# nabeelre/BTSbot

Hardware: AMD Instinct MI355X
Metric: alerts/sec (63×63×3 triplet + 25 meta) train+infer, 1/2/4/8 MI355X (higher is better)
Workload: dtype bf16; 1 GPU; BASELINE.json configs[1]: ConvNeXt-pico multi-modal (mm_ConvNeXt) bf16 inference, batch=1024 synthetic triplets per GPU, inputs resident in HBM, logits+scores out; per_gpu_batch=1024, global_batch=1024, precision=bf16, weights=seeded random, layer-scale ~1, parallelism=1 independent replicas, batch-sharded, no collective, pipeline_depth=3

## Files before the change

### btsbot_amd/csrc/stage1b.hip

```cpp
#include "common.h"
#include "stage0.h"
#include <type_traits>

namespace {

typedef __attribute__((ext_vector_type(16))) float f32x16;
typedef __attribute__((address_space(1))) const void* gptr_t;
typedef __attribute__((address_space(3))) void* lptr_t;

template <typename T> struct SCM;
typedef __attribute__((ext_vector_type(4))) short s16x4;
typedef __attribute__((ext_vector_type(4))) _Float16 f16x4;
template <> struct SCM<bf16_t> {
  using frag = bf16x8;
  using frag4 = s16x4;
  static __device__ __forceinline__ f32x16 run(frag a, frag b, f32x16 c) {
    return __builtin_amdgcn_mfma_f32_32x32x16_bf16(a, b, c, 0, 0, 0);
  }
  static __device__ __forceinline__ f32x4 run4(frag4 a, frag4 b, f32x4 c) {
    return __builtin_amdgcn_mfma_f32_4x4x4bf16_1k(a, b, c, 0, 0, 0);
  }
};
template <> struct SCM<f16_t> {
  using frag = f16x8;
  using frag4 = f16x4;
  static __device__ __forceinline__ f32x16 run(frag a, frag b, f32x16 c) {
    return __builtin_amdgcn_mfma_f32_32x32x16_f16(a, b, c, 0, 0, 0);
  }
  static __device__ __forceinline__ f32x4 run4(frag4 a, frag4 b, f32x4 c) {
    return __builtin_amdgcn_mfma_f32_4x4x4f16(a, b, c, 0, 0, 0);
  }
};

constexpr int C = 128, HW = 7, PA = 49, G = 2, NPX = G * PA, CT = 4, HID = 512, KS1 = 8;
constexpr int CN = 256, PO = 9;
constexpr int PITCH = 2 * C + 16;
constexpr int MAPB = NPX * PITCH;
constexpr int CHUNKB = 16384, HALFB = CHUNKB / 2, NCH = HID / 32, NSLOT = 3;
constexpr int PL_ROW = 136 * 8, PL_XQ = 8 * PL_ROW, PL_AL = 2 * PL_XQ, PLB = G * PL_AL;
constexpr int OFF_PL = 2 * CHUNKB;
template <bool X2> struct S1L {
  static constexpr int PLANES = X2 ? 2 : 1;
  static constexpr int SLB = X2 ? 2 * HALFB : HALFB;
  static constexpr int OFF_W2X = OFF_PL + PLANES * PLB;
  static constexpr int OFF_B1 = OFF_W2X + (X2 ? 2 * SLB : 0);
  static constexpr int OFF_PART = OFF_B1 + (HID + C) * 4;
  static constexpr int OFF_ST = OFF_PART + 2 * 4 * 128 * 4;
  static constexpr int LDS_BYTES = OFF_ST + 2 * 128 * 4;
  static_assert(4 * SLB <= PLANES * PLB, "W1 slots + W2 slot 0 inside the planar images");
};
static_assert(MAPB <= 2 * CHUNKB && S1L<false>::LDS_BYTES <= 80 * 1024 && S1L<true>::LDS_BYTES <= 160 * 1024, "LDS layout");
constexpr float LN_EPS = 1e-6f;
constexpr int TW_R = 21, TW_BYTES = TW_R * C * 4 * 4 * 2;
constexpr int PARB = TW_BYTES + 3 * C * 4;
constexpr int PARB_X2 = 2 * TW_BYTES + 3 * C * 4;

#define SC_STAMP(i)                                                                \
  do {                                                                             \
    if (a.stamps != nullptr && blockIdx.x == 0 && threadIdx.x == 0) a.stamps[i] = clock64(); \
    if (a.wgt != nullptr && threadIdx.x == 0 && ((i) == 0 || (i) == 13))           \
      a.wgt[2 * blockIdx.x + ((i) == 13)] = wall_clock64();                        \
  } while (0)

template <int N> __device__ __forceinline__ void wait_vm() {
  asm volatile("s_waitcnt vmcnt(%0)" ::"n"(N) : "memory");
}
__device__ __forceinline__ int swz4(int row) {
  return (4 - ((row >> 2) & 3)) & 3;
}
__device__ __forceinline__ float swap_add32(float a, float b) {
  auto r = __builtin_amdgcn_permlane32_swap(__float_as_uint(a), __float_as_uint(b), false, false);
  return __uint_as_float(r[0]) + __uint_as_float(r[1]);
}
__device__ __forceinline__ float swap_add16(float a, float b) {
  auto r = __builtin_amdgcn_permlane16_swap(__float_as_uint(a), __float_as_uint(b), false, false);
  return __uint_as_float(r[0]) + __uint_as_float(r[1]);
}
template <int CTRL> __device__ __forceinline__ float dpp_mov(float v) {
  return __builtin_bit_cast(float, __builtin_amdgcn_update_dpp(0, __builtin_bit_cast(int, v), CTRL, 0xF, 0xF, true));
}
__device__ __forceinline__ void block_reduce32(float (&w)[32], int lane, float (&out)[2]) {
#pragma unroll
  for (int n = 0; n < 16; ++n) w[n] = swap_add32(w[n], w[n + 16]);
#pragma unroll
  for (int n = 0; n < 8; ++n) w[n] = swap_add16(w[n], w[n + 8]);
  const bool b3 = (lane & 8) != 0, b2 = (lane & 4) != 0;
#pragma unroll
  for (int n = 0; n < 4; ++n) {
    const float own = b3 ? w[n + 4] : w[n], send = b3 ? w[n] : w[n + 4];
    w[n] = own + dpp_mov<0x128>(send);
  }
#pragma unroll
  for (int n = 0; n < 2; ++n) {
    const float own = b2 ? w[n + 2] : w[n], send = b2 ? w[n] : w[n + 2];
    const float lo = dpp_mov<0x124>(send), hi = dpp_mov<0x12C>(send);
    out[n] = own + (b2 ? lo : hi);
  }
}

__device__ __forceinline__ void ln_regs(const f32x16 (&x)[CT], const float* __restrict__ w,
                                        const float* __restrict__ b, int h, f32x16 (&y)[CT]) {
  float s = 0.f;
#pragma unroll
  for (int ct = 0; ct < CT; ++ct)
#pragma unroll
    for (int r = 0; r < 16; ++r) s += x[ct][r];
  s += __shfl_xor(s, 32, 64);
  const float mean = s * (1.0f / C);
  float q = 0.f;
#pragma unroll
  for (int ct = 0; ct < CT; ++ct)
#pragma unroll
    for (int r = 0; r < 16; ++r) {
      const float d = x[ct][r] - mean;
      q += d * d;
    }
  q += __shfl_xor(q, 32, 64);
  const float rstd = rsqrtf(q * (1.0f / C) + LN_EPS);
#pragma unroll
  for (int ct = 0; ct < CT; ++ct)
#pragma unroll
    for (int qd = 0; qd < 4; ++qd) {
      const int c = ct * 32 + 8 * qd + 4 * h;
      const float4 wv = *reinterpret_cast<const float4*>(w + c);
      const float4 bv = *reinterpret_cast<const float4*>(b + c);
      y[ct][4 * qd + 0] = (x[ct][4 * qd + 0] - mean) * rstd * wv.x + bv.x;
      y[ct][4 * qd + 1] = (x[ct][4 * qd + 1] - mean) * rstd * wv.y + bv.y;
      y[ct][4 * qd + 2] = (x[ct][4 * qd + 2] - mean) * rstd * wv.z + bv.z;
      y[ct][4 * qd + 3] = (x[ct][4 * qd + 3] - mean) * rstd * wv.w + bv.w;
    }
}

template <typename T, int LOPLANE = 0>
__device__ __forceinline__ void regs_to_map(const f32x16 (&x)[CT], unsigned char* map, int p, int h) {
  typedef T __attribute__((ext_vector_type(4))) T4;
#pragma unroll
  for (int ct = 0; ct < CT; ++ct)
#pragma unroll
    for (int qd = 0; qd < 4; ++qd) {
      T4 v, w;
#pragma unroll
      for (int e = 0; e < 4; ++e) {
        v[e] = (T)x[ct][4 * qd + e];
        if (LOPLANE > 0) w[e] = (T)(x[ct][4 * qd + e] - (float)v[e]);
      }
      *reinterpret_cast<T4*>(map + p * PITCH + (ct * 32 + 8 * qd + 4 * h) * 2) = v;
      if (LOPLANE > 0) *reinterpret_cast<T4*>(map + LOPLANE + p * PITCH + (ct * 32 + 8 * qd + 4 * h) * 2) = w;
    }
}

template <typename T, int LOPLANE = 0, bool SAT = false>
__device__ __forceinline__ void regs_to_planar(const f32x16 (&x)[CT], unsigned char* pl, int p, int h) {
  const int al = p >= PA ? 1 : 0, pp = p - al * PA;
  const int y = pp / HW, xx = pp - y * HW;
  unsigned char* dst = pl + al * PL_AL + (xx >> 2) * PL_XQ + y * PL_ROW + (xx & 3) * 2 + h * 32;
#pragma unroll
  for (int ct = 0; ct < CT; ++ct)
#pragma unroll
    for (int r = 0; r < 16; ++r) {
      const T hi = (T)(SAT ? __builtin_amdgcn_fmed3f(x[ct][r], -65504.0f, 65504.0f) : x[ct][r]);
      *reinterpret_cast<T*>(dst + (ct * 32 + 8 * (r >> 2) + (r & 3)) * 8) = hi;
      if (LOPLANE > 0) *reinterpret_cast<T*>(dst + LOPLANE + (ct * 32 + 8 * (r >> 2) + (r & 3)) * 8) = (T)(x[ct][r] - (float)hi);
    }
}

template <typename T, bool X2, int WPS = 2, bool KEEP = false>
__global__ __launch_bounds__(256, WPS) void stage1b_kernel(Stage1Args a) {
  using frag = typename SCM<T>::frag;
  using DT = typename std::conditional<KEEP, f16_t, T>::type;
  using frag4 = typename SCM<DT>::frag4;
  extern __shared__ __attribute__((aligned(16))) unsigned char smem[];
  unsigned char* pl = smem + OFF_PL;
  unsigned char* stg = smem;
  using L = S1L<X2>;
  constexpr int SLB = L::SLB;
  constexpr int PLO = X2 ? PLB : 0;
  float* b1s = reinterpret_cast<float*>(smem + L::OFF_B1);
  float* b2s = b1s + HID;
  float* part = reinterpret_cast<float*>(smem + L::OFF_PART);
  float* st = reinterpret_cast<float*>(smem + L::OFF_ST);
  auto w1slot = [&](int sl) { return pl + sl * SLB; };
  auto w2slot = [&](int sl) { return sl == 0 ? pl + 3 * SLB : (X2 ? smem + L::OFF_W2X : smem) + (sl - 1) * SLB; };

  const int tid = threadIdx.x, lane = tid & 63, wave = __builtin_amdgcn_readfirstlane(tid >> 6);
  const int lr = lane & 31, h = lane >> 5;
  const bool w1wave = wave < 2;
  const int a0 = blockIdx.x * G;
  const int nal = min(G, a.B - a0);
  const int p = wave * 32 + lr;
  const bool live = p < nal * PA;
  const bool inmap = p < NPX;
  const int pm = inmap ? p : 0;
  SC_STAMP(0);
  auto zero_pads = [&]() {
#pragma unroll
    for (int pn = 0; pn < L::PLANES; ++pn) {
      unsigned char* pb = pl + pn * PLB;
      for (int i = tid; i < 4 * PL_ROW / 16; i += 256) {
        const int blk = i / (PL_ROW / 16), o = i - blk * (PL_ROW / 16);
        *reinterpret_cast<uint4*>(pb + (blk >> 1) * PL_AL + (blk & 1) * PL_XQ + 7 * PL_ROW + o * 16) = make_uint4(0u, 0u, 0u, 0u);
      }
      for (int i = tid; i < G * HW * C; i += 256) {
        const int al = i / (HW * C), r = (i / C) % HW, c = i % C;
        *reinterpret_cast<unsigned short*>(pb + al * PL_AL + PL_XQ + r * PL_ROW + c * 8 + 6) = 0;
      }
    }
  };
  zero_pads();
  const float* xsrc = a.x_in + ((size_t)a0 * PA + (live ? p : 0)) * C;
  float* xscr = a.scratch + ((size_t)a0 * PA + (live ? p : 0)) * C;
  auto load_x = [&](const float* src, f32x16 (&x)[CT]) {
#pragma unroll
    for (int ct = 0; ct < CT; ++ct)
#pragma unroll
      for (int qd = 0; qd < 4; ++qd) {
        const float4 v4 = *reinterpret_cast<const float4*>(src + ct * 32 + 8 * qd + 4 * h);
        x[ct][4 * qd + 0] = live ? v4.x : 0.f;
        x[ct][4 * qd + 1] = live ? v4.y : 0.f;
        x[ct][4 * qd + 2] = live ? v4.z : 0.f;
        x[ct][4 * qd + 3] = live ? v4.w : 0.f;
      }
  };
  {
    f32x16 x0[CT];
    load_x(xsrc, x0);
    if (inmap) regs_to_planar<DT, PLO, KEEP && !std::is_same<T, f16_t>::value>(x0, pl, p, h);
  }
  SC_STAMP(1);

  f32x16 x[CT];
  const int rot = (blockIdx.x * 5 + (blockIdx.x >> 4)) & (NCH - 1);
#pragma unroll
  for (int j = 0; j < 2; ++j) {
    const Stage0Blk& bk = a.blk[j];
    int ln = lane;
    asm volatile("" : "+v"(ln));
    const int dj = ln & 3, db = ln >> 2;
    const float b1v0 = bk.b1[tid], b1v1 = bk.b1[256 + tid];
    const float b2v = bk.gamma[tid & (C - 1)] * bk.b2[tid & (C - 1)];
    const uint2* twsrc = reinterpret_cast<const uint2*>(bk.par) + (2 * wave) * 64 + ln;
    frag4 tw[TW_R], twl[X2 ? TW_R : 1];
#pragma unroll
    for (int r = 0; r < TW_R; ++r) tw[r] = __builtin_bit_cast(frag4, twsrc[r * 512]);
    if (X2) {
#pragma unroll
      for (int r = 0; r < TW_R; ++r) twl[r] = __builtin_bit_cast(frag4, twsrc[TW_BYTES / 8 + r * 512]);
    }
    const float* pf = reinterpret_cast<const float*>(bk.par + (X2 ? 2 : 1) * TW_BYTES);
    float dwbias[2], lng[2], lnb2[2];
#pragma unroll
    for (int gi = 0; gi < 2; ++gi) {
      const int c = 16 * (2 * wave + gi) + db;
      dwbias[gi] = pf[c];
      lng[gi] = pf[C + c];
      lnb2[gi] = pf[2 * C + c];
    }
    SC_STAMP(2 + 5 * j);
    __syncthreads();
    b1s[tid] = b1v0;
    b1s[256 + tid] = b1v1;
    if (tid < C) b2s[tid] = b2v;

    const unsigned char* wsrc[4];
    const unsigned char* wsrcl[4];
#pragma unroll
    for (int i = 0; i < 4; ++i) {
      const int pc = wave * 4 + i;
      if (pc < 8) {
        const int m = pc * 4 + (lane >> 4);
        const int hid = (m & ~12) | ((m & 4) << 1) | ((m & 8) >> 1);
        const size_t o = (size_t)hid * (C * 2) + (((lane & 15) ^ (m & 15)) << 4);
        wsrc[i] = bk.w1 + o;
        wsrcl[i] = X2 ? bk.w1_lo + o : nullptr;
      } else {
        const int r = (pc - 8) * 16 + (lane >> 2);
        const size_t o = (size_t)r * (HID * 2) + (((lane & 3) ^ swz4(r)) << 4);
        wsrc[i] = bk.w2g + o;
        wsrcl[i] = X2 ? bk.w2g_lo + o : nullptr;
      }
    }
    const int wstep0 = w1wave ? 32 * C * 2 : 64;
    auto issue = [&](int k) {
      unsigned char* dst = (w1wave ? w1slot(k % NSLOT) : w2slot(k % NSLOT)) + (wave & 1) * 4096;
#pragma unroll
      for (int i = 0; i < 4; ++i)
        __builtin_amdgcn_global_load_lds((gptr_t)(wsrc[i] + (size_t)((k + rot) & (NCH - 1)) * wstep0),
                                         (lptr_t)(dst + i * 1024), 16, 0, 0);
      if (X2) {
#pragma unroll
        for (int i = 0; i < 4; ++i)
          __builtin_amdgcn_global_load_lds((gptr_t)(wsrcl[i] + (size_t)((k + rot) & (NCH - 1)) * wstep0),
                                           (lptr_t)(dst + HALFB + i * 1024), 16, 0, 0);
      }
    };
    auto issue_piece = [&](int k, int i) {
      unsigned char* dst = (w1wave ? w1slot(k % NSLOT) : w2slot(k % NSLOT)) + (wave & 1) * 4096;
      if (X2 && i >= 4)
        __builtin_amdgcn_global_load_lds((gptr_t)(wsrcl[i & 3] + (size_t)((k + rot) & (NCH - 1)) * wstep0),
                                         (lptr_t)(dst + HALFB + (i & 3) * 1024), 16, 0, 0);
      else
        __builtin_amdgcn_global_load_lds((gptr_t)(wsrc[i] + (size_t)((k + rot) & (NCH - 1)) * wstep0),
                                         (lptr_t)(dst + i * 1024), 16, 0, 0);
    };
    SC_STAMP(3 + 5 * j);

    int rofs[11];
#pragma unroll
    for (int sx = 0; sx < 11; ++sx) {
      const int r = sx + dj - 3;
      rofs[sx] = ((unsigned)r < (unsigned)HW ? r : 7) * PL_ROW;
    }
    float v[2][2][16];
#pragma unroll
    for (int gi = 0; gi < 2; ++gi) {
      if (gi == 1) {
#pragma unroll
        for (int r = 0; r < TW_R; ++r) tw[r] = __builtin_bit_cast(frag4, twsrc[r * 512 + 64]);
        if (X2) {
#pragma unroll
          for (int r = 0; r < TW_R; ++r) twl[r] = __builtin_bit_cast(frag4, twsrc[TW_BYTES / 8 + r * 512 + 64]);
        }
      }
      f32x4 acc[G][2][2];
#pragma unroll
      for (int al = 0; al < G; ++al)
#pragma unroll
        for (int yb = 0; yb < 2; ++yb)
#pragma unroll
          for (int xb = 0; xb < 2; ++xb) acc[al][yb][xb] = f32x4{dwbias[gi], dwbias[gi], dwbias[gi], dwbias[gi]};
      const unsigned char* lb = pl + (16 * (2 * wave + gi) + db) * 8;
      frag4 bq[2][G][2], bql[X2 ? 2 : 1][G][X2 ? 2 : 1];
      auto read_step = [&](int sx, int buf) {
#pragma unroll
        for (int al = 0; al < G; ++al)
#pragma unroll
          for (int q = 0; q < 2; ++q) {
            bq[buf][al][q] = __builtin_bit_cast(frag4, *reinterpret_cast<const uint2*>(lb + al * PL_AL + q * PL_XQ + rofs[sx]));
            if (X2)
              bql[buf][al][q] =
                  __builtin_bit_cast(frag4, *reinterpret_cast<const uint2*>(lb + PLB + al * PL_AL + q * PL_XQ + rofs[sx]));
          }
      };
      read_step(0, 0);
#ifdef S1_EXP_NODW
#pragma unroll 1
      for (int sx = 0; sx < 0; ++sx) {
#else
#pragma unroll
      for (int sx = 0; sx < 11; ++sx) {
#endif
#pragma unroll
        for (int al = 0; al < G; ++al)
#pragma unroll
          for (int q = 0; q < 2; ++q) {
            asm volatile("" : "+v"(bq[sx & 1][al][q]));
            if (X2) asm volatile("" : "+v"(bql[X2 ? sx & 1 : 0][al][X2 ? q : 0]));
          }
        if (sx + 1 < 11) read_step(sx + 1, (sx + 1) & 1);
        __builtin_amdgcn_sched_barrier(0);
#pragma unroll
        for (int al = 0; al < G; ++al)
#pragma unroll
          for (int yb = 0; yb < 2; ++yb) {
            const int ky = sx - 4 * yb;
            if (ky < 0 || ky > 6) continue;
#pragma unroll
            for (int rbi = 0; rbi < 3; ++rbi)
#pragma unroll
              for (int xb = 0; xb < 2; ++xb) {
                const int q = xb + rbi - 1;
                if (q < 0 || q > 1) continue;
                if (X2) {
                  acc[al][yb][xb] = SCM<DT>::run4(twl[ky * 3 + rbi], bq[sx & 1][al][q], acc[al][yb][xb]);
                  acc[al][yb][xb] = SCM<DT>::run4(tw[ky * 3 + rbi], bql[X2 ? sx & 1 : 0][al][X2 ? q : 0], acc[al][yb][xb]);
                }
                acc[al][yb][xb] = SCM<DT>::run4(tw[ky * 3 + rbi], bq[sx & 1][al][q], acc[al][yb][xb]);
              }
          }
        __builtin_amdgcn_sched_barrier(0);
      }
#pragma unroll
      for (int al = 0; al < G; ++al)
#pragma unroll
        for (int yb = 0; yb < 2; ++yb)
#pragma unroll
          for (int xb = 0; xb < 2; ++xb)
#pragma unroll
            for (int i = 0; i < 4; ++i) v[gi][al][yb * 8 + xb * 4 + i] = acc[al][yb][xb][i];
    }
    if (KEEP && a.keep_d[j] != nullptr) {
#pragma unroll
      for (int gi = 0; gi < 2; ++gi)
#pragma unroll
        for (int al = 0; al < G; ++al) {
          if (al >= nal) continue;
          float* dst = a.keep_d[j] + (size_t)(a0 + al) * PA * C + 16 * (2 * wave + gi) + db;
#pragma unroll
          for (int yb = 0; yb < 2; ++yb)
#pragma unroll
            for (int xb = 0; xb < 2; ++xb)
              if (yb < 1 || dj < 3) {
#pragma unroll
                for (int i = 0; i < 4; ++i) {
                  if (xb == 1 && i == 3) continue;
                  dst[((4 * yb + dj) * HW + 4 * xb + i) * C] = v[gi][al][yb * 8 + xb * 4 + i];
                }
              }
        }
    }
    SC_STAMP(4 + 5 * j);
    {
      float o1[2], o2[2];
      {
        float s1[32];
#pragma unroll
        for (int al = 0; al < G; ++al)
#pragma unroll
          for (int n = 0; n < 16; ++n) s1[al * 16 + n] = v[0][al][n] + v[1][al][n];
        block_reduce32(s1, ln, o1);
      }
      {
        float s2[32];
#pragma unroll
        for (int al = 0; al < G; ++al)
#pragma unroll
          for (int n = 0; n < 16; ++n) s2[al * 16 + n] = fmaf(v[0][al][n], v[0][al][n], v[1][al][n] * v[1][al][n]);
        block_reduce32(s2, ln, o2);
      }
      const int slot = (ln >> 5) * 64 + (4 * ((ln >> 4) & 1) + dj) * 8 + 4 * ((ln >> 3) & 1) + 2 * ((ln >> 2) & 1);
      *reinterpret_cast<float2*>(part + wave * 128 + slot) = make_float2(o1[0], o1[1]);
      *reinterpret_cast<float2*>(part + 512 + wave * 128 + slot) = make_float2(o2[0], o2[1]);
    }
    __syncthreads();
    if (tid < 128) {
      const float t1 = part[tid] + part[128 + tid] + part[256 + tid] + part[384 + tid];
      const float t2 = part[512 + tid] + part[640 + tid] + part[768 + tid] + part[896 + tid];
      const float mean = t1 * (1.0f / C);
      const float rstd = rsqrtf(fmaxf(t2 * (1.0f / C) - mean * mean, 0.0f) + LN_EPS);
      st[tid] = rstd;
      st[128 + tid] = -mean * rstd;
    }
    __syncthreads();
    auto write_ln = [&](bool lo_pass) {
#pragma unroll
      for (int gi = 0; gi < 2; ++gi) {
        T* mo = reinterpret_cast<T*>(stg) + 16 * (2 * wave + gi) + db;
#pragma unroll
        for (int al = 0; al < G; ++al)
#pragma unroll
          for (int yb = 0; yb < 2; ++yb)
#pragma unroll
            for (int xb = 0; xb < 2; ++xb) {
              const int slot = al * 64 + (4 * yb + dj) * 8 + 4 * xb;
              const float4 r4 = *reinterpret_cast<const float4*>(st + slot);
              const float4 m4 = *reinterpret_cast<const float4*>(st + 128 + slot);
              const float rr[4] = {r4.x, r4.y, r4.z, r4.w}, mm[4] = {m4.x, m4.y, m4.z, m4.w};
              if (yb < 1 || dj < 3) {
#pragma unroll
                for (int i = 0; i < 4; ++i) {
                  if (xb == 1 && i == 3) continue;
                  const float y = fmaf(fmaf(v[gi][al][yb * 8 + xb * 4 + i], rr[i], mm[i]), lng[gi], lnb2[gi]);
                  const T yh = (T)y;
                  mo[(al * PA + (4 * yb + dj) * HW + 4 * xb + i) * (PITCH / 2)] = lo_pass ? (T)(y - (float)yh) : yh;
                }
              }
            }
      }
    };
    write_ln(false);
    __syncthreads();
    if (KEEP) {
      unsigned char* dst = reinterpret_cast<unsigned char*>(a.keep_xn[j]) + (size_t)a0 * PA * C * 2;
      for (int i = tid; i < nal * PA * 16; i += 256) {
        const int pp = i >> 4, c16 = i & 15;
        *reinterpret_cast<uint4*>(dst + (size_t)pp * C * 2 + 16 * c16) = *reinterpret_cast<const uint4*>(stg + pp * PITCH + 16 * c16);
      }
    }
    issue(0);
    SC_STAMP(5 + 5 * j);

    load_x(j == 0 ? xsrc : xscr, x);
    {
      frag xf[KS1], xfl[X2 ? KS1 : 1];
#pragma unroll
      for (int ks = 0; ks < KS1; ++ks)
        xf[ks] = *reinterpret_cast<const frag*>(stg + pm * PITCH + ks * 32 + h * 16);
      if (X2) {
        __syncthreads();
        write_ln(true);
        __syncthreads();
#pragma unroll
        for (int ks = 0; ks < KS1; ++ks)
          xfl[ks] = *reinterpret_cast<const frag*>(stg + pm * PITCH + ks * 32 + h * 16);
      }
#pragma unroll
      for (int ct = 0; ct < CT; ++ct)
#pragma unroll
        for (int qd = 0; qd < 4; ++qd) {
          const float4 bv = *reinterpret_cast<const float4*>(b2s + ct * 32 + 8 * qd + 4 * h);
          x[ct][4 * qd + 0] += bv.x;
          x[ct][4 * qd + 1] += bv.y;
          x[ct][4 * qd + 2] += bv.z;
          x[ct][4 * qd + 3] += bv.w;
        }
      asm volatile("s_waitcnt lgkmcnt(0)" ::: "memory");
      __syncthreads();
      issue(1);
      if (w1wave) issue(2);
      auto bias_acc = [&](int k, f32x16& acc) {
        const float* bp = b1s + ((k + rot) & (NCH - 1)) * 32 + 8 * h;
#pragma unroll
        for (int qd = 0; qd < 4; ++qd) {
          const f32x4 bv = __builtin_bit_cast(f32x4, *reinterpret_cast<const bf16x8*>(bp + 4 * (qd & 1) + 16 * (qd >> 1)));
#pragma unroll
          for (int e = 0; e < 4; ++e) acc[4 * qd + e] = bv[e];
        }
      };
      frag a1l[X2 ? KS1 : 1];
      auto read_a1 = [&](int k, frag (&a1)[KS1]) {
        const unsigned char* w1s = w1slot(k % NSLOT);
#pragma unroll
        for (int ks = 0; ks < KS1; ++ks) {
          a1[ks] = *reinterpret_cast<const frag*>(w1s + lr * 256 + (((ks * 2 + h) ^ (lr & 15)) << 4));
          if (X2) a1l[ks] = *reinterpret_cast<const frag*>(w1s + HALFB + lr * 256 + (((ks * 2 + h) ^ (lr & 15)) << 4));
        }
      };
#ifdef S1_LOOPSTAMP
      unsigned long long lts[16];
#define LS(i) do { __builtin_amdgcn_sched_barrier(0); if (ch == 6 || ch == 7) lts[i + 8 * (ch - 6)] = __builtin_amdgcn_s_memtime(); __builtin_amdgcn_sched_barrier(0); } while (0)
#else
#define LS(i)
#endif
      f32x16 hacc[2];
      frag a1[KS1];
      {
        wait_vm<X2 ? 8 : 4>();
        asm volatile("s_waitcnt lgkmcnt(0)" ::: "memory");
        __builtin_amdgcn_s_barrier();
        bias_acc(0, hacc[0]);
        read_a1(0, a1);
#pragma unroll
        for (int ks = 0; ks < KS1; ++ks) {
          if (X2) {
            hacc[0] = SCM<T>::run(a1l[ks], xf[ks], hacc[0]);
            hacc[0] = SCM<T>::run(a1[ks], xfl[ks], hacc[0]);
          }
          hacc[0] = SCM<T>::run(a1[ks], xf[ks], hacc[0]);
        }
        __builtin_amdgcn_sched_barrier(0);
        wait_vm<0>();
        asm volatile("s_waitcnt lgkmcnt(0)" ::: "memory");
        __builtin_amdgcn_s_barrier();
        bias_acc(1, hacc[1]);
        read_a1(1, a1);
        if (w1wave) issue(3);
      }
      auto step = [&](auto last_c, int ch, f32x16& hc, f32x16& hn) {
        constexpr bool LAST = decltype(last_c)::value;
        LS(0);
        wait_vm<X2 ? 8 : 4>();
        LS(1);
        asm volatile("s_waitcnt lgkmcnt(0)" ::: "memory");
#ifndef S1_EXP_NOBAR
        __builtin_amdgcn_s_barrier();
#endif
        LS(2);
        frag a2[CT][2], a2l[X2 ? CT : 1][2];
        const unsigned char* w2s = w2slot(ch % NSLOT);
#pragma unroll
        for (int ct = 0; ct < CT; ++ct)
#pragma unroll
          for (int s2 = 0; s2 < 2; ++s2) {
            const int r = ct * 32 + lr;
            a2[ct][s2] = *reinterpret_cast<const frag*>(w2s + r * 64 + (((s2 * 2 + h) ^ swz4(r)) << 4));
            if (X2) a2l[ct][s2] = *reinterpret_cast<const frag*>(w2s + HALFB + r * 64 + (((s2 * 2 + h) ^ swz4(r)) << 4));
          }
        LS(3);
        const int kdma = ch + (w1wave ? 4 : 2);
        __builtin_amdgcn_sched_barrier(0);
        LS(4);
        float g[16];
#pragma unroll
        for (int r = 0; r < 8; ++r) {
          if (!LAST) {
            if (X2) {
              hn = SCM<T>::run(a1l[r], xf[r], hn);
              hn = SCM<T>::run(a1[r], xfl[r], hn);
            }
            hn = SCM<T>::run(a1[r], xf[r], hn);
          }
#ifdef S1_EXP_NOGELU
          g[r] = hc[r];
#else
          g[r] = gelu_for<T>(hc[r]);
#endif
#ifndef S1_EXP_NODMA
          if (X2) issue_piece(kdma, r);
          else if (r & 1) issue_piece(kdma, r >> 1);
#endif
          __builtin_amdgcn_sched_barrier(0);
        }
        LS(5);
        if (!LAST) read_a1(ch + 2, a1);
        frag hf, hfl;
#pragma unroll
        for (int r = 0; r < 8; ++r) {
          hf[r] = (T)g[r];
          if (X2) hfl[r] = (T)(g[r] - (float)hf[r]);
        }
#pragma unroll
        for (int ct = 0; ct < CT; ++ct) {
          if (X2) {
            x[ct] = SCM<T>::run(a2l[ct][0], hf, x[ct]);
            x[ct] = SCM<T>::run(a2[ct][0], hfl, x[ct]);
          }
          x[ct] = SCM<T>::run(a2[ct][0], hf, x[ct]);
#ifdef S1_EXP_NOGELU
          g[8 + 2 * ct] = hc[8 + 2 * ct];
          g[9 + 2 * ct] = hc[9 + 2 * ct];
#else
          g[8 + 2 * ct] = gelu_for<T>(hc[8 + 2 * ct]);
          g[9 + 2 * ct] = gelu_for<T>(hc[9 + 2 * ct]);
#endif
          __builtin_amdgcn_sched_barrier(0);
        }
        if (!LAST) bias_acc(ch + 2, hc);
#pragma unroll
        for (int r = 0; r < 8; ++r) {
          hf[r] = (T)g[8 + r];
          if (X2) hfl[r] = (T)(g[8 + r] - (float)hf[r]);
        }
        LS(6);
#pragma unroll
        for (int ct = 0; ct < CT; ++ct) {
          if (X2) {
            x[ct] = SCM<T>::run(a2l[ct][1], hf, x[ct]);
            x[ct] = SCM<T>::run(a2[ct][1], hfl, x[ct]);
          }
          x[ct] = SCM<T>::run(a2[ct][1], hf, x[ct]);
        }
        LS(7);
      };
#ifndef S1_EXP_NOLOOP
#pragma unroll 1
      for (int ch = 0; ch < NCH - 2; ch += 2) {
        step(std::false_type{}, ch, hacc[0], hacc[1]);
        step(std::false_type{}, ch + 1, hacc[1], hacc[0]);
      }
      step(std::false_type{}, NCH - 2, hacc[0], hacc[1]);
      step(std::true_type{}, NCH - 1, hacc[1], hacc[0]);
#endif
      asm volatile("s_waitcnt lgkmcnt(0)" ::: "memory");
#ifdef S1_LOOPSTAMP
      if (a.wgt != nullptr && blockIdx.x == 0 && tid == 0 && j == 0)
        for (int i = 0; i < 16; ++i) a.wgt[4096 + i] = lts[i];
#endif
      wait_vm<0>();
      if (j == 0) {
        __syncthreads();
        zero_pads();
        if (inmap) regs_to_planar<DT, PLO, KEEP && !std::is_same<T, f16_t>::value>(x, pl, p, h);
        if (live) {
#pragma unroll
          for (int ct = 0; ct < CT; ++ct)
#pragma unroll
            for (int qd = 0; qd < 4; ++qd)
              *reinterpret_cast<float4*>(xscr + ct * 32 + 8 * qd + 4 * h) =
                  make_float4(x[ct][4 * qd], x[ct][4 * qd + 1], x[ct][4 * qd + 2], x[ct][4 * qd + 3]);
        }
      }
    }
    SC_STAMP(6 + 5 * j);
  }
  if (a.tap_stage != nullptr && live) {
    float* tp = a.tap_stage + ((size_t)a0 * PA + p) * C;
#pragma unroll
    for (int ct = 0; ct < CT; ++ct)
#pragma unroll
      for (int qd = 0; qd < 4; ++qd)
        *reinterpret_cast<float4*>(tp + ct * 32 + 8 * qd + 4 * h) =
            make_float4(x[ct][4 * qd], x[ct][4 * qd + 1], x[ct][4 * qd + 2], x[ct][4 * qd + 3]);
  }

  {
    __syncthreads();
    {
      f32x16 xn[CT];
      ln_regs(x, a.ds_lnw, a.ds_lnb, h, xn);
      if (inmap) regs_to_map<T, X2 ? MAPB : 0>(xn, stg, p, h);
    }
    static_assert(2 * MAPB <= L::OFF_B1, "two [pixel][channel] images in front of the bias words");
    constexpr int KSD = 4 * C / 16, RING = X2 ? 8 : 16, NSTEP = 2 * KSD;
    const frag* wsrc = reinterpret_cast<const frag*>(a.ds_w) + lane;
    auto fsrc = [&](int stp) {
      return wsrc + (size_t)((wave + 4 * (stp >> 5)) * KSD + (stp & (KSD - 1))) * (X2 ? 128 : 64);
    };
    frag wq[RING], wql[X2 ? RING : 1];
#pragma unroll
    for (int i = 0; i < RING; ++i) {
      wq[i] = *fsrc(i);
      if (X2) wql[i] = fsrc(i)[64];
    }
    __syncthreads();
    if (KEEP) {
      unsigned char* dst = reinterpret_cast<unsigned char*>(a.keep_patches) + (size_t)a0 * PO * 4 * C * 2;
      for (int i = tid; i < nal * PO * 4 * 16; i += 256) {
        const int c16 = i & 15, q = (i >> 4) & 3, o2 = i >> 6;
        const int g2 = o2 / PO, oo2 = o2 - g2 * PO;
        const int pin2 = g2 * PA + (2 * (oo2 / 3) + (q >> 1)) * HW + 2 * (oo2 % 3) + (q & 1);
        *reinterpret_cast<uint4*>(dst + (size_t)(o2 * 4 + q) * C * 2 + 16 * c16) =
            *reinterpret_cast<const uint4*>(stg + pin2 * PITCH + 16 * c16);
      }
    }
    SC_STAMP(12);
    const int o = lr;
    const bool olive = o < nal * PO;
    const int oc = o < G * PO ? o : 0;
    const int g = oc / PO, oo = oc - g * PO;
    const int oy = oo / 3, ox = oo - oy * 3;
    f32x16 acc;
    constexpr int RPT = KSD / RING;
#ifdef S1_EXP_NODS
#pragma unroll 1
    for (int rd = 0; rd < 0; ++rd) {
#else
#pragma unroll 1
    for (int rd = 0; rd < NSTEP / RING; ++rd) {
#endif
      const int cot = wave + 4 * (rd / RPT);
      if (rd % RPT == 0) {
#pragma unroll
        for (int qd = 0; qd < 4; ++qd) {
          const float4 bv = *reinterpret_cast<const float4*>(a.ds_b + cot * 32 + 8 * qd + 4 * h);
          acc[4 * qd + 0] = bv.x;
          acc[4 * qd + 1] = bv.y;
          acc[4 * qd + 2] = bv.z;
          acc[4 * qd + 3] = bv.w;
        }
      }
#pragma unroll
      for (int i = 0; i < RING; ++i) {
        const int stp = rd * RING + i, ks = stp & (KSD - 1);
        const int q = ks >> 3;
        const int pin = g * PA + (2 * oy + (q >> 1)) * HW + 2 * ox + (q & 1);
        const frag bf = *reinterpret_cast<const frag*>(stg + pin * PITCH + (ks & 7) * 32 + h * 16);
        if (X2) {
          const frag bfl = *reinterpret_cast<const frag*>(stg + MAPB + pin * PITCH + (ks & 7) * 32 + h * 16);
          acc = SCM<T>::run(wql[i], bf, acc);
          acc = SCM<T>::run(wq[i], bfl, acc);
        }
        acc = SCM<T>::run(wq[i], bf, acc);
        if (stp + RING < NSTEP) {
          wq[i] = *fsrc(stp + RING);
          if (X2) wql[i] = fsrc(stp + RING)[64];
        }
      }
      if (rd % RPT == RPT - 1 && olive) {
        float* dst = a.out + ((size_t)a0 * PO + o) * CN + cot * 32 + 4 * h;
#pragma unroll
        for (int qd = 0; qd < 4; ++qd)
          *reinterpret_cast<float4*>(dst + 8 * qd) =
              make_float4(acc[4 * qd], acc[4 * qd + 1], acc[4 * qd + 2], acc[4 * qd + 3]);
      }
    }
    SC_STAMP(13);
  }
}

template <typename T, bool X2>
__global__ void pack_s1par_kernel(const float* __restrict__ taps, const float* __restrict__ dw_b,
                                  const float* __restrict__ ln_w, const float* __restrict__ ln_b,
                                  unsigned char* __restrict__ out) {
  const int idx = blockIdx.x * blockDim.x + threadIdx.x;
  constexpr int NTW = TW_R * C * 16;
  if (idx < NTW) {
    const int k = idx & 3, i = (idx >> 2) & 3, c = (idx >> 4) & (C - 1), r = idx / (16 * C);
    const int ky = r / 3, rb = r % 3 - 1, kx = 4 * rb + k - i + 3;
    const float w = (kx >= 0 && kx < 7) ? taps[(ky * 7 + kx) * C + c] : 0.f;
    const T wh = (T)w;
    reinterpret_cast<T*>(out)[idx] = wh;
    if (X2) reinterpret_cast<T*>(out)[NTW + idx] = (T)(w - (float)wh);
    return;
  }
  const int f = idx - NTW;
  if (f >= 3 * C) return;
  float v;
  if (f < C) v = dw_b[f];
  else if (f < 2 * C) v = ln_w[f - C];
  else v = ln_b[f - 2 * C];
  reinterpret_cast<float*>(out + (X2 ? 2 : 1) * TW_BYTES)[f] = v;
}

template <typename T, bool X2 = false>
__global__ void pack_frag32_kernel(const float* __restrict__ w, T* __restrict__ out, int rows, int cin) {
  const long i = (long)blockIdx.x * blockDim.x + threadIdx.x;
  const int K = 4 * cin;
  if (i >= (long)rows * K) return;
  const int j = (int)(i & 7), l = (int)((i >> 3) & 63);
  const long fs = i >> 9;
  const int ksteps = K / 16;
  const int sk = (int)(fs % ksteps), tile = (int)(fs / ksteps);
  const int row = 32 * tile + (l & 31), k = 16 * sk + 8 * (l >> 5) + j;
  const int q = k / cin, c = k - q * cin;
  const float v = w[((long)row * cin + c) * 4 + q];
  const T vh = (T)v;
  if (X2) {
    out[fs * 1024 + l * 8 + j] = vh;
    out[fs * 1024 + 512 + l * 8 + j] = (T)(v - (float)vh);
  } else {
    out[i] = vh;
  }
}

template <typename T, bool X2 = false, int WPS = 2, bool KEEP = false> int launch_stage1b_t(const Stage1Args& a, hipStream_t st) {
  auto kern = stage1b_kernel<T, X2, WPS, KEEP>;
  static DevOnce attr_set;
  static const int pad = switch_on(SW_S1_ONE_WG) && !X2 ? 90 * 1024 - S1L<X2>::LDS_BYTES : 0;
  const int LDS_BYTES = S1L<X2>::LDS_BYTES + pad;
  if (attr_set.need()) {
    HIP_TRY(hipFuncSetAttribute(reinterpret_cast<const void*>(kern),
                                hipFuncAttributeMaxDynamicSharedMemorySize, (int)LDS_BYTES));
    attr_set.done();
  }
  hipLaunchKernelGGL(kern, dim3((a.B + G - 1) / G), dim3(256), LDS_BYTES, st, a);
  LAUNCH_CHECK();
  return BTSBOT_OK;
}

}

#ifdef STAGE1B_X2_TU
int launch_stage1b_x2(const Stage1Args& a, hipStream_t st) {
  if (a.blk[0].w1_lo == nullptr || a.blk[0].w2g_lo == nullptr || a.blk[1].w1_lo == nullptr || a.blk[1].w2g_lo == nullptr) {
    btsbot_set_error("stage1b: the split mode needs the filters' remainder images (w1_lo, w2g_lo)");
    return BTSBOT_ERR_INVALID_ARG;
  }
  return launch_stage1b_t<f16_t, true, 1>(a, st);
}
int launch_pack_s1par_x2(const float* taps, const float* dw_b, const float* ln_w, const float* ln_b, void* out,
                         hipStream_t st) {
  const dim3 grid((TW_R * C * 16 + 3 * C + 255) / 256), blk(256);
  hipLaunchKernelGGL((pack_s1par_kernel<f16_t, true>), grid, blk, 0, st, taps, dw_b, ln_w, ln_b,
                     reinterpret_cast<unsigned char*>(out));
  LAUNCH_CHECK();
  return BTSBOT_OK;
}
int launch_pack_frag32_x2(const float* src, void* dst, int cout, int cin, hipStream_t st) {
  const long total = (long)cout * 4 * cin;
  hipLaunchKernelGGL((pack_frag32_kernel<f16_t, true>), dim3((unsigned)((total + 255) / 256)), dim3(256), 0, st, src,
                     reinterpret_cast<f16_t*>(dst), cout, cin);
  LAUNCH_CHECK();
  return BTSBOT_OK;
}
#else
int launch_stage1b_x2(const Stage1Args& a, hipStream_t st);
int launch_pack_s1par_x2(const float* taps, const float* dw_b, const float* ln_w, const float* ln_b, void* out,
                         hipStream_t st);
int launch_pack_frag32_x2(const float* src, void* dst, int cout, int cin, hipStream_t st);

size_t s1par_bytes() { return PARB_X2; }

int launch_pack_s1par(int prec, const float* taps, const float* dw_b, const float* ln_w,
                      const float* ln_b, void* out, hipStream_t st) {
  unsigned char* o = reinterpret_cast<unsigned char*>(out);
  const dim3 grid((TW_R * C * 16 + 3 * C + 255) / 256), blk(256);
  if (prec == BTSBOT_BF16)
    hipLaunchKernelGGL((pack_s1par_kernel<bf16_t, false>), grid, blk, 0, st, taps, dw_b, ln_w, ln_b, o);
  else if (prec == BTSBOT_F16)
    hipLaunchKernelGGL((pack_s1par_kernel<f16_t, false>), grid, blk, 0, st, taps, dw_b, ln_w, ln_b, o);
  else if (prec == BTSBOT_F16X2)
    return launch_pack_s1par_x2(taps, dw_b, ln_w, ln_b, out, st);
  else {
    btsbot_set_error("pack_s1par: precision %d is not a 16-bit mode", prec);
    return BTSBOT_ERR_INVALID_ARG;
  }
  LAUNCH_CHECK();
  return BTSBOT_OK;
}

int launch_pack_frag32(int prec, const float* src, void* dst, int cout, int cin, hipStream_t st) {
  const long total = (long)cout * 4 * cin;
  const dim3 grid((unsigned)((total + 255) / 256)), blk(256);
  if (prec == BTSBOT_BF16)
    hipLaunchKernelGGL(pack_frag32_kernel<bf16_t>, grid, blk, 0, st, src, reinterpret_cast<bf16_t*>(dst), cout, cin);
  else if (prec == BTSBOT_F16)
    hipLaunchKernelGGL(pack_frag32_kernel<f16_t>, grid, blk, 0, st, src, reinterpret_cast<f16_t*>(dst), cout, cin);
  else if (prec == BTSBOT_F16X2)
    return launch_pack_frag32_x2(src, dst, cout, cin, st);
  else {
    btsbot_set_error("pack_frag32: precision %d is not a 16-bit mode", prec);
    return BTSBOT_ERR_INVALID_ARG;
  }
  LAUNCH_CHECK();
  return BTSBOT_OK;
}

bool stage1_supported(int prec, int c1, int c2) {
  return (prec == BTSBOT_BF16 || prec == BTSBOT_F16 || prec == BTSBOT_F16X2) && c1 == 128 && c2 == 256;
}

int launch_stage1b(int prec, const Stage1Args& a, hipStream_t st) {
  if (a.B <= 0) return BTSBOT_OK;
  if (a.keep_xn[0] != nullptr) {
    if ((a.keep_d[0] == nullptr) != (a.keep_d[1] == nullptr) || a.keep_xn[1] == nullptr || a.keep_patches == nullptr ||
        a.tap_stage == nullptr || a.scratch == nullptr) {
      btsbot_set_error("stage1b: the training forward needs every kept buffer");
      return BTSBOT_ERR_INVALID_ARG;
    }
    if (prec == BTSBOT_BF16) return launch_stage1b_t<bf16_t, false, 2, true>(a, st);
    if (prec == BTSBOT_F16) return launch_stage1b_t<f16_t, false, 2, true>(a, st);
    btsbot_set_error("stage1b: the training forward runs in the bf16 / f16 modes, not %d", prec);
    return BTSBOT_ERR_INVALID_ARG;
  }
  if (prec == BTSBOT_BF16) return launch_stage1b_t<bf16_t>(a, st);
  if (prec == BTSBOT_F16) return launch_stage1b_t<f16_t>(a, st);
  if (prec == BTSBOT_F16X2) return launch_stage1b_x2(a, st);
  btsbot_set_error("stage1b: unsupported precision %d", prec);
  return BTSBOT_ERR_INVALID_ARG;
}
#endif
```

Baseline: 3.637 million alerts/s.

## Move ConvNeXt LayerNorm into per-pixel registers after fp32 LDS transpose

The depthwise-conv output is no longer reduced across lanes with permlane/DPP and a partial-sum table. It is now written as an fp32 image into LDS, reusing the ring slots and planar area. Each lane reads back its pixel's 64 channels and computes mean and variance in registers, then builds the bf16 MFMA fragments and the optional low-precision residual fragments directly. This removes extra barriers and the staging write/read of normalized activations. The residual x load is deferred and overlapped with the first W1 chunk by raising the vmcnt wait threshold, and LN weights move to LDS. In exchange it writes and reads a larger fp32 image in LDS, raises register pressure (64 floats plus 16 float4 per lane), and uses two-pass variance instead of E[x²]-mean².

```diff
diff --git a/btsbot_amd/csrc/stage1b.hip b/btsbot_amd/csrc/stage1b.hip
--- a/btsbot_amd/csrc/stage1b.hip
+++ b/btsbot_amd/csrc/stage1b.hip
@@ -39,17 +39,18 @@
 constexpr int CHUNKB = 16384, HALFB = CHUNKB / 2, NCH = HID / 32, NSLOT = 3;
 constexpr int PL_ROW = 136 * 8, PL_XQ = 8 * PL_ROW, PL_AL = 2 * PL_XQ, PLB = G * PL_AL;
 constexpr int OFF_PL = 2 * CHUNKB;
+constexpr int LNP = 4 * C + 16;
 template <bool X2> struct S1L {
   static constexpr int PLANES = X2 ? 2 : 1;
   static constexpr int SLB = X2 ? 2 * HALFB : HALFB;
   static constexpr int OFF_W2X = OFF_PL + PLANES * PLB;
   static constexpr int OFF_B1 = OFF_W2X + (X2 ? 2 * SLB : 0);
-  static constexpr int OFF_PART = OFF_B1 + (HID + C) * 4;
-  static constexpr int OFF_ST = OFF_PART + 2 * 4 * 128 * 4;
-  static constexpr int LDS_BYTES = OFF_ST + 2 * 128 * 4;
+  static constexpr int OFF_LNW = OFF_B1 + (HID + C) * 4;
+  static constexpr int LDS_BYTES = OFF_LNW + 2 * C * 4;
   static_assert(4 * SLB <= PLANES * PLB, "W1 slots + W2 slot 0 inside the planar images");
+  static_assert(NPX * LNP <= OFF_PL + PLB && NPX * LNP <= OFF_B1, "the fp32 image lies in ring slots 0, 1 + the planar image");
 };
-static_assert(MAPB <= 2 * CHUNKB && S1L<false>::LDS_BYTES <= 80 * 1024 && S1L<true>::LDS_BYTES <= 160 * 1024, "LDS layout");
+static_assert(MAPB <= 2 * CHUNKB && S1L<false>::LDS_BYTES <= 75264 && S1L<true>::LDS_BYTES <= 160 * 1024, "LDS layout");
 constexpr float LN_EPS = 1e-6f;
 constexpr int TW_R = 21, TW_BYTES = TW_R * C * 4 * 4 * 2;
 constexpr int PARB = TW_BYTES + 3 * C * 4;
@@ -68,36 +69,6 @@
 __device__ __forceinline__ int swz4(int row) {
   return (4 - ((row >> 2) & 3)) & 3;
 }
-__device__ __forceinline__ float swap_add32(float a, float b) {
-  auto r = __builtin_amdgcn_permlane32_swap(__float_as_uint(a), __float_as_uint(b), false, false);
-  return __uint_as_float(r[0]) + __uint_as_float(r[1]);
-}
-__device__ __forceinline__ float swap_add16(float a, float b) {
-  auto r = __builtin_amdgcn_permlane16_swap(__float_as_uint(a), __float_as_uint(b), false, false);
-  return __uint_as_float(r[0]) + __uint_as_float(r[1]);
-}
-template <int CTRL> __device__ __forceinline__ float dpp_mov(float v) {
-  return __builtin_bit_cast(float, __builtin_amdgcn_update_dpp(0, __builtin_bit_cast(int, v), CTRL, 0xF, 0xF, true));
-}
-__device__ __forceinline__ void block_reduce32(float (&w)[32], int lane, float (&out)[2]) {
-#pragma unroll
-  for (int n = 0; n < 16; ++n) w[n] = swap_add32(w[n], w[n + 16]);
-#pragma unroll
-  for (int n = 0; n < 8; ++n) w[n] = swap_add16(w[n], w[n + 8]);
-  const bool b3 = (lane & 8) != 0, b2 = (lane & 4) != 0;
-#pragma unroll
-  for (int n = 0; n < 4; ++n) {
-    const float own = b3 ? w[n + 4] : w[n], send = b3 ? w[n] : w[n + 4];
-    w[n] = own + dpp_mov<0x128>(send);
-  }
-#pragma unroll
-  for (int n = 0; n < 2; ++n) {
-    const float own = b2 ? w[n + 2] : w[n], send = b2 ? w[n] : w[n + 2];
-    const float lo = dpp_mov<0x124>(send), hi = dpp_mov<0x12C>(send);
-    out[n] = own + (b2 ? lo : hi);
-  }
-}
-
 __device__ __forceinline__ void ln_regs(const f32x16 (&x)[CT], const float* __restrict__ w,
                                         const float* __restrict__ b, int h, f32x16 (&y)[CT]) {
   float s = 0.f;
@@ -177,8 +148,8 @@
   constexpr int PLO = X2 ? PLB : 0;
   float* b1s = reinterpret_cast<float*>(smem + L::OFF_B1);
   float* b2s = b1s + HID;
-  float* part = reinterpret_cast<float*>(smem + L::OFF_PART);
-  float* st = reinterpret_cast<float*>(smem + L::OFF_ST);
+  float* lnws = reinterpret_cast<float*>(smem + L::OFF_LNW);
+  float* lnbs = lnws + C;
   auto w1slot = [&](int sl) { return pl + sl * SLB; };
   auto w2slot = [&](int sl) { return sl == 0 ? pl + 3 * SLB : (X2 ? smem + L::OFF_W2X : smem) + (sl - 1) * SLB; };
 
@@ -191,6 +162,7 @@
   const bool live = p < nal * PA;
   const bool inmap = p < NPX;
   const int pm = inmap ? p : 0;
+  const int lnrow = pm * LNP + h * 32;
   SC_STAMP(0);
   auto zero_pads = [&]() {
 #pragma unroll
@@ -247,19 +219,16 @@
       for (int r = 0; r < TW_R; ++r) twl[r] = __builtin_bit_cast(frag4, twsrc[TW_BYTES / 8 + r * 512]);
     }
     const float* pf = reinterpret_cast<const float*>(bk.par + (X2 ? 2 : 1) * TW_BYTES);
-    float dwbias[2], lng[2], lnb2[2];
-#pragma unroll
-    for (int gi = 0; gi < 2; ++gi) {
-      const int c = 16 * (2 * wave + gi) + db;
-      dwbias[gi] = pf[c];
-      lng[gi] = pf[C + c];
-      lnb2[gi] = pf[2 * C + c];
-    }
+    float dwbias[2];
+#pragma unroll
+    for (int gi = 0; gi < 2; ++gi) dwbias[gi] = pf[16 * (2 * wave + gi) + db];
+    const float lnv = pf[C + tid];
     SC_STAMP(2 + 5 * j);
     __syncthreads();
     b1s[tid] = b1v0;
     b1s[256 + tid] = b1v1;
     if (tid < C) b2s[tid] = b2v;
+    lnws[tid] = lnv;
 
     const unsigned char* wsrc[4];
     const unsigned char* wsrcl[4];
@@ -409,104 +378,86 @@
         }
     }
     SC_STAMP(4 + 5 * j);
+    __syncthreads();
     {
-      float o1[2], o2[2];
-      {
-        float s1[32];
+      unsigned char* dst = smem + dj * (HW * LNP) + (32 * wave + db) * 4;
+#pragma unroll
+      for (int gi = 0; gi < 2; ++gi)
 #pragma unroll
         for (int al = 0; al < G; ++al)
 #pragma unroll
-          for (int n = 0; n < 16; ++n) s1[al * 16 + n] = v[0][al][n] + v[1][al][n];
-        block_reduce32(s1, ln, o1);
-      }
-      {
-        float s2[32];
-#pragma unroll
-        for (int al = 0; al < G; ++al)
-#pragma unroll
-          for (int n = 0; n < 16; ++n) s2[al * 16 + n] = fmaf(v[0][al][n], v[0][al][n], v[1][al][n] * v[1][al][n]);
-        block_reduce32(s2, ln, o2);
-      }
-      const int slot = (ln >> 5) * 64 + (4 * ((ln >> 4) & 1) + dj) * 8 + 4 * ((ln >> 3) & 1) + 2 * ((ln >> 2) & 1);
-      *reinterpret_cast<float2*>(part + wave * 128 + slot) = make_float2(o1[0], o1[1]);
-      *reinterpret_cast<float2*>(part + 512 + wave * 128 + slot) = make_float2(o2[0], o2[1]);
-    }
-    __syncthreads();
-    if (tid < 128) {
-      const float t1 = part[tid] + part[128 + tid] + part[256 + tid] + part[384 + tid];
-      const float t2 = part[512 + tid] + part[640 + tid] + part[768 + tid] + part[896 + tid];
-      const float mean = t1 * (1.0f / C);
-      const float rstd = rsqrtf(fmaxf(t2 * (1.0f / C) - mean * mean, 0.0f) + LN_EPS);
-      st[tid] = rstd;
-      st[128 + tid] = -mean * rstd;
-    }
-    __syncthreads();
-    auto write_ln = [&](bool lo_pass) {
-#pragma unroll
-      for (int gi = 0; gi < 2; ++gi) {
-        T* mo = reinterpret_cast<T*>(stg) + 16 * (2 * wave + gi) + db;
-#pragma unroll
-        for (int al = 0; al < G; ++al)
-#pragma unroll
           for (int yb = 0; yb < 2; ++yb)
 #pragma unroll
-            for (int xb = 0; xb < 2; ++xb) {
-              const int slot = al * 64 + (4 * yb + dj) * 8 + 4 * xb;
-              const float4 r4 = *reinterpret_cast<const float4*>(st + slot);
-              const float4 m4 = *reinterpret_cast<const float4*>(st + 128 + slot);
-              const float rr[4] = {r4.x, r4.y, r4.z, r4.w}, mm[4] = {m4.x, m4.y, m4.z, m4.w};
+            for (int xb = 0; xb < 2; ++xb)
               if (yb < 1 || dj < 3) {
 #pragma unroll
                 for (int i = 0; i < 4; ++i) {
                   if (xb == 1 && i == 3) continue;
-                  const float y = fmaf(fmaf(v[gi][al][yb * 8 + xb * 4 + i], rr[i], mm[i]), lng[gi], lnb2[gi]);
-                  const T yh = (T)y;
-                  mo[(al * PA + (4 * yb + dj) * HW + 4 * xb + i) * (PITCH / 2)] = lo_pass ? (T)(y - (float)yh) : yh;
+                  const int col = 4 * xb + i, ofs = (al * PA + 4 * yb * HW + col) * LNP + gi * 64;
+                  *reinterpret_cast<float*>(dst + ofs) = v[gi][al][yb * 8 + xb * 4 + i];
                 }
               }
-            }
-      }
-    };
-    write_ln(false);
+    }
     __syncthreads();
-    if (KEEP) {
-      unsigned char* dst = reinterpret_cast<unsigned char*>(a.keep_xn[j]) + (size_t)a0 * PA * C * 2;
-      for (int i = tid; i < nal * PA * 16; i += 256) {
-        const int pp = i >> 4, c16 = i & 15;
-        *reinterpret_cast<uint4*>(dst + (size_t)pp * C * 2 + 16 * c16) = *reinterpret_cast<const uint4*>(stg + pp * PITCH + 16 * c16);
-      }
-    }
-    issue(0);
-    SC_STAMP(5 + 5 * j);
-
-    load_x(j == 0 ? xsrc : xscr, x);
+
     {
+      auto lds4 = [](const void* q) { return __builtin_bit_cast(f32x4, *reinterpret_cast<const bf16x8*>(q)); };
       frag xf[KS1], xfl[X2 ? KS1 : 1];
+      float xv[64];
 #pragma unroll
       for (int ks = 0; ks < KS1; ++ks)
-        xf[ks] = *reinterpret_cast<const frag*>(stg + pm * PITCH + ks * 32 + h * 16);
-      if (X2) {
-        __syncthreads();
-        write_ln(true);
-        __syncthreads();
-#pragma unroll
-        for (int ks = 0; ks < KS1; ++ks)
-          xfl[ks] = *reinterpret_cast<const frag*>(stg + pm * PITCH + ks * 32 + h * 16);
-      }
-#pragma unroll
-      for (int ct = 0; ct < CT; ++ct)
-#pragma unroll
-        for (int qd = 0; qd < 4; ++qd) {
-          const float4 bv = *reinterpret_cast<const float4*>(b2s + ct * 32 + 8 * qd + 4 * h);
-          x[ct][4 * qd + 0] += bv.x;
-          x[ct][4 * qd + 1] += bv.y;
-          x[ct][4 * qd + 2] += bv.z;
-          x[ct][4 * qd + 3] += bv.w;
+#pragma unroll
+        for (int q = 0; q < 2; ++q) {
+          const f32x4 r4 = lds4(smem + lnrow + ks * 64 + q * 16);
+#pragma unroll
+          for (int e = 0; e < 4; ++e) xv[ks * 8 + q * 4 + e] = r4[e];
         }
       asm volatile("s_waitcnt lgkmcnt(0)" ::: "memory");
-      __syncthreads();
+      __builtin_amdgcn_s_barrier();
+      issue(0);
       issue(1);
       if (w1wave) issue(2);
+      float s = 0.f;
+#pragma unroll
+      for (int n = 0; n < 64; ++n) s += xv[n];
+      s += __shfl_xor(s, 32, 64);
+      const float mean = s * (1.0f / C);
+      float q2 = 0.f;
+#pragma unroll
+      for (int n = 0; n < 64; ++n) {
+        xv[n] -= mean;
+        q2 += xv[n] * xv[n];
+      }
+      q2 += __shfl_xor(q2, 32, 64);
+      const float rstd = rsqrtf(q2 * (1.0f / C) + LN_EPS);
+#pragma unroll
+      for (int ks = 0; ks < KS1; ++ks) {
+#pragma unroll
+        for (int q = 0; q < 2; ++q) {
+          const f32x4 w4 = lds4(lnws + ks * 16 + h * 8 + q * 4), b4 = lds4(lnbs + ks * 16 + h * 8 + q * 4);
+#pragma unroll
+          for (int e = 0; e < 4; ++e) {
+            const float y = xv[ks * 8 + q * 4 + e] * rstd * w4[e] + b4[e];
+            const T yh = (T)y;
+            xf[ks][q * 4 + e] = yh;
+            if (X2) xfl[X2 ? ks : 0][q * 4 + e] = (T)(y - (float)yh);
+          }
+        }
+        if (KEEP && live)
+          *reinterpret_cast<frag*>(reinterpret_cast<unsigned char*>(a.keep_xn[j]) + ((size_t)a0 * PA + p) * C * 2 + ks * 32 +
+                                   h * 16) = xf[ks];
+      }
+      SC_STAMP(5 + 5 * j);
+      float4 xt[4 * CT];
+      __builtin_amdgcn_sched_barrier(0);
+      {
+        const float* src = j == 0 ? xsrc : xscr;
+#pragma unroll
+        for (int ct = 0; ct < CT; ++ct)
+#pragma unroll
+          for (int qd = 0; qd < 4; ++qd) xt[4 * ct + qd] = *reinterpret_cast<const float4*>(src + ct * 32 + 8 * qd + 4 * h);
+      }
+      __builtin_amdgcn_sched_barrier(0);
       auto bias_acc = [&](int k, f32x16& acc) {
         const float* bp = b1s + ((k + rot) & (NCH - 1)) * 32 + 8 * h;
 #pragma unroll
@@ -534,7 +485,7 @@
       f32x16 hacc[2];
       frag a1[KS1];
       {
-        wait_vm<X2 ? 8 : 4>();
+        wait_vm<(X2 ? 8 : 4) + 16>();
         asm volatile("s_waitcnt lgkmcnt(0)" ::: "memory");
         __builtin_amdgcn_s_barrier();
         bias_acc(0, hacc[0]);
@@ -553,6 +504,21 @@
         __builtin_amdgcn_s_barrier();
         bias_acc(1, hacc[1]);
         read_a1(1, a1);
+        __builtin_amdgcn_sched_barrier(0);
+#pragma unroll
+        for (int ct = 0; ct < CT; ++ct)
+#pragma unroll
+          for (int qd = 0; qd < 4; ++qd) {
+            const f32x4 bv = lds4(b2s + ct * 32 + 8 * qd + 4 * h);
+            const float4 v4 = xt[4 * ct + qd];
+            x[ct][4 * qd + 0] = (live ? v4.x : 0.f) + bv[0];
+            x[ct][4 * qd + 1] = (live ? v4.y : 0.f) + bv[1];
+            x[ct][4 * qd + 2] = (live ? v4.z : 0.f) + bv[2];
+            x[ct][4 * qd + 3] = (live ? v4.w : 0.f) + bv[3];
+          }
+#pragma unroll
+        for (int ct = 0; ct < CT; ++ct) asm volatile("" : "+v"(x[ct]));
+        __builtin_amdgcn_sched_barrier(0);
         if (w1wave) issue(3);
       }
       auto step = [&](auto last_c, int ch, f32x16& hc, f32x16& hn) {
```

Measured after the change: 3.733 million alerts/s (median of 6 runs). 2.7% higher.
